# robflynnyh/long-context-asr

Measured on AMD Instinct MI355X. Metric: spectrogram-frames/sec (6L/768D, seq=16384), higher is better.
Workload: dtype bf16; 1 GPU; 6L/768D/6H SConformerXL, seq=16384, rotary theta=1.5M, fwd+CTC+bwd+clip+MADGRAD; per_gpu_batch=128, global_batch=128, seq_len=16384, parallelism=dp1

## Files before the change

long-context-asr_amd/csrc/convmod.hip:

```cpp
#include "common.h"

namespace {

constexpr int CV = 4;

struct SlabGeo {
    int cg, sl, cpb, spb;
    bool active;
    __device__ __forceinline__ SlabGeo(int CG) {
        cpb = min(64, CG); spb = 256 / cpb;
        const int cgl = threadIdx.x % cpb;
        sl = threadIdx.x / cpb;
        cg = blockIdx.y * cpb + cgl;
        active = cg < CG && sl < spb;
    }
};
template <typename AT>
__device__ __forceinline__ void slab_reduce_add(const float (&v)[CV], const SlabGeo& g, float* sh, AT* out, int d, long det_stride) {
    __syncthreads();
    if (threadIdx.x < g.cpb * g.spb) {
#pragma unroll
        for (int e = 0; e < CV; ++e) sh[g.sl * (g.cpb * CV) + (threadIdx.x % g.cpb) * CV + e] = g.active ? v[e] : 0.f;
    }
    __syncthreads();
// ... 186 lines not shown
    const long slab = (long)blockIdx.x * geo.spb + geo.sl;
    const bool live = geo.active && slab < (long)B * spb;
    const int b = live ? (int)(slab / spb) : 0, n0 = live ? (int)(slab % spb) * TN : 0;
    const int c0 = live ? geo.cg * CV : 0;
    const int L = len ? len[b] : N;
    float wk[K][CV], dhw[K][CV], aw[K][CV], gw[K][CV], gb[CV];
    float sv[CV] = {0.f, 0.f, 0.f, 0.f}, sg2[CV] = {0.f, 0.f, 0.f, 0.f};
    float mean[CV], is[CV], A[CV], Bc[CV], k0[CV], k1[CV], k2[CV];
    load4(coef + c0, mean); load4(coef + d + c0, is); load4(coef + 4 * d + c0, A); load4(coef + 5 * d + c0, Bc);
    load4(bcoef + c0, k0); load4(bcoef + d + c0, k1); load4(bcoef + 2 * d + c0, k2);
#pragma unroll
    for (int e = 0; e < CV; ++e) {
        is[e] = 1.f / is[e]; gb[e] = 0.f;
#pragma unroll
        for (int j = 0; j < K; ++j) { wk[j][e] = w[(c0 + e) * K + j]; dhw[j][e] = 0.f; aw[j][e] = 0.f; gw[j][e] = 0.f; }
    }
    const bf16* gbp = g + (long)b * N * 2 * d;
    const int nend = live ? min(N, n0 + TN) : n0 - 2 * P;
    struct Raw { bf16x4 gy, hx, va, ga, cva, cga; };
    const bf16x4 z4 = {(bf16)0.f, (bf16)0.f, (bf16)0.f, (bf16)0.f};
    auto fetch = [&](int t) {
        Raw r; r.gy = z4; r.hx = z4; r.va = z4; r.ga = z4; r.cva = z4; r.cga = z4;
        if (t >= 0 && t < N) {
            const long row = (long)b * N + t;
            r.gy = *reinterpret_cast<const bf16x4*>(dy + row * d + c0);
            r.hx = *reinterpret_cast<const bf16x4*>(h + row * d + c0);
            if (t < L) {
                r.va = *reinterpret_cast<const bf16x4*>(gbp + (long)t * 2 * d + c0);
                r.ga = *reinterpret_cast<const bf16x4*>(gbp + (long)t * 2 * d + d + c0);
            }
        }
        const int n = t - P;
        if (n >= n0 && n < nend && n < L) {
            r.cva = *reinterpret_cast<const bf16x4*>(gbp + (long)n * 2 * d + c0);
            r.cga = *reinterpret_cast<const bf16x4*>(gbp + (long)n * 2 * d + d + c0);
        }
        return r;
    };
    Raw cur = fetch(n0 - P);
    for (int t = n0 - P; t < nend + P; ++t) {
        const Raw nxt = fetch(t + 1 < nend + P ? t + 1 : -1000000);
#pragma unroll
        for (int j = 0; j < K - 1; ++j)
#pragma unroll
            for (int e = 0; e < CV; ++e) { dhw[j][e] = dhw[j + 1][e]; aw[j][e] = aw[j + 1][e]; }
        if (t >= 0 && t < N) {
#pragma unroll
            for (int e = 0; e < CV; ++e) {
                const float hx = (float)cur.hx[e];
                const float dz = (float)cur.gy[e] * dsiluf_(hx * A[e] + Bc[e]);
                dhw[K - 1][e] = k0[e] * dz - k1[e] - (hx - mean[e]) * is[e] * k2[e];
                aw[K - 1][e] = (t < L) ? (float)cur.va[e] * sigmoidf_((float)cur.ga[e]) : 0.f;
            }
        } else {
#pragma unroll
            for (int e = 0; e < CV; ++e) { dhw[K - 1][e] = 0.f; aw[K - 1][e] = 0.f; }
        }
        const int n = t - P;
        if (n >= n0 && n < nend) {
            float dv[CV], dgt[CV];
#pragma unroll
            for (int e = 0; e < CV; ++e) {
                float acc = 0.f;
                const float dhc = dhw[P][e];
#pragma unroll
                for (int j = 0; j < K; ++j) { acc += wk[j][e] * dhw[K - 1 - j][e]; gw[j][e] += dhc * aw[j][e]; }
                gb[e] += dhc;
                if (n < L) {
                    const float sg = sigmoidf_((float)cur.cga[e]);
                    dv[e] = acc * sg; dgt[e] = acc * (float)cur.cva[e] * sg * (1.f - sg);
                } else { dv[e] = 0.f; dgt[e] = 0.f; }
                sv[e] += dv[e]; sg2[e] += dgt[e];
            }
            bf16* o = dg + ((long)b * N + n) * 2 * d;
            store4(o + c0, dv); store4(o + d + c0, dgt);
        }
        cur = nxt;
    }
    slab_reduce_add<float>(gb, geo, redw, dbias, d, det_stride);
#pragma unroll
    for (int j = 0; j < K; ++j) slab_reduce_add<float>(gw[j], geo, redw, dwt + (long)j * d, d, det_stride);
    if (dgcs) { slab_reduce_add<float>(sv, geo, redw, dgcs, d, det_stride); slab_reduce_add<float>(sg2, geo, redw, dgcs + d, d, det_stride); }
}

int pick_tn(long B, long N, long CG) {
    int TN = 64;
    while (TN > 8 && B * cdiv(N, TN) * CG < 131072) TN >>= 1;
    return TN;
}

}

static dim3 glu_fwd_grid(long B, long N, long d, int& TN) {
    TN = pick_tn(B, N, d / CV);
    const int cpb = (int)std::min<long>(64, d / CV), spbk = 256 / cpb;
    return dim3(cdiv(B * cdiv(N, TN), spbk), cdiv(d / CV, cpb));
}
SCONF_API int64_t sconf_glu_dwconv_fwd_workspace(int64_t B, int64_t N, int64_t d) {
    if (B * N == 0 || d % CV != 0) return 0;
    int TN; return (int64_t)glu_fwd_grid(B, N, d, TN).x * 2 * d * 8;
}
SCONF_API int sconf_glu_dwconv_fwd(const void* g, const int32_t* lengths, const float* w, const float* bias, void* h,
                                   double* stats, void* workspace, int64_t workspace_bytes, int64_t B, int64_t N, int64_t d,
                                   int64_t ksize, hipStream_t stream) {
    SCONF_REQUIRE(d % CV == 0, "sconf_glu_dwconv_fwd: d must be a multiple of 4");
    if (B * N == 0) return 0;
    int TN;
    const dim3 grid = glu_fwd_grid(B, N, d, TN), block(256);
    SCONF_REQUIRE(ksize == 3 || ksize == 5 || ksize == 7 || ksize == 9, "sconf_glu_dwconv_fwd: unsupported kernel size %ld (3,5,7,9)", (long)ksize);
    double* sl = stats ? det_begin<double>(workspace, workspace_bytes, grid.x, 2 * d, stream) : nullptr;
    SCONF_REQUIRE(!stats || sl, "sconf_glu_dwconv_fwd: needs %ld bytes of workspace (sconf_glu_dwconv_fwd_workspace)",
                  (long)sconf_glu_dwconv_fwd_workspace(B, N, d));
#define L(KK) hipLaunchKernelGGL((glu_dwconv_fwd_kernel<KK>), grid, block, 0, stream, (const bf16*)g, lengths, w, bias, (bf16*)h, sl, (int)B, (int)N, (int)d, TN, 2 * d)
    switch (ksize) { case 3: L(3); break; case 5: L(5); break; case 7: L(7); break; default: L(9); break; }
#undef L
    if (stats) det_finish<double>(sl, grid.x, 2 * d, DetSegs<double>{{stats}, {0}, {2 * d}, 1}, stream);
    SCONF_LAUNCH_OK("sconf_glu_dwconv_fwd");
    return 0;
}

SCONF_API int sconf_brn_finalize(const double* stats, int64_t count, float* running_mean, float* running_std,
                                 int64_t* num_batches_tracked, const float* weight, const float* bias, float* coef,
                                 int64_t d, int training, float eps, float momentum, hipStream_t stream) {
    hipLaunchKernelGGL(brn_finalize_kernel, dim3(cdiv(d, 256)), dim3(256), 0, stream, stats, (double)count, running_mean,
                       running_std, (long*)num_batches_tracked, weight, bias, coef, (int)d, training, eps, momentum);
    if (training) hipLaunchKernelGGL(brn_bump_kernel, dim3(1), dim3(64), 0, stream, (long*)num_batches_tracked);
    SCONF_LAUNCH_OK("sconf_brn_finalize");
    return 0;
}

SCONF_API int sconf_affine_silu_fwd(const void* h, const float* coef, void* y, int64_t M, int64_t d, hipStream_t stream) {
    SCONF_REQUIRE(d % 8 == 0, "sconf_affine_silu_fwd: d must be a multiple of 8");
    if (M == 0) return 0;
    const int blocks = (int)std::min<long>(cdiv(M * (d / 8), 256), 8192);
    hipLaunchKernelGGL(affine_silu_fwd_kernel, dim3(blocks), dim3(256), 0, stream, (const bf16*)h, coef, (bf16*)y, (long)M, (int)d);
    SCONF_LAUNCH_OK("sconf_affine_silu_fwd");
    return 0;
}

struct ConvmodBwdGeo { int rpt, cpb, spbk, rrows, TN; dim3 grid; long gst; };
static ConvmodBwdGeo convmod_bwd_geo(long B, long N, long d, long ksize, bool colsum) {
    ConvmodBwdGeo q;
    const long M = B * N;
    const int CG = (int)(d / CV);
    q.rpt = 64;
    while (q.rpt > 8 && cdiv(M, q.rpt) * CG < 131072) q.rpt >>= 1;
    q.cpb = std::min(64, CG); q.spbk = 256 / q.cpb;
    q.rrows = cdiv(cdiv(M, q.rpt), q.spbk);
    q.TN = pick_tn(B, N, CG);
    q.grid = dim3(cdiv(B * cdiv(N, q.TN), q.spbk), cdiv(CG, q.cpb));
    q.gst = d + ksize * d + (colsum ? 2 * d : 0);
    return q;
}
SCONF_API int sconf_convmod_tile_frames(int64_t B, int64_t N, int64_t d) {
    if (B <= 0 || N <= 0 || d <= 0 || d % CV != 0) return -1;
    return pick_tn(B, N, d / CV);
}
SCONF_API int sconf_convmod_bwd_rows_per_thread(int64_t B, int64_t N, int64_t d) {
    if (B <= 0 || N <= 0 || d <= 0 || d % CV != 0) return -1;
    return convmod_bwd_geo(B, N, d, 9, false).rpt;
}
SCONF_API int64_t sconf_convmod_bwd_workspace(int64_t B, int64_t N, int64_t d, int64_t ksize, int colsum) {
    if (B * N == 0 || d % CV != 0) return 0;
    const ConvmodBwdGeo q = convmod_bwd_geo(B, N, d, ksize, colsum != 0);
    return std::max<int64_t>((int64_t)q.rrows * 2 * d * 8, (int64_t)q.grid.x * q.gst * 4);
}
SCONF_API int sconf_convmod_bwd(const void* dy, const void* h, const void* g, const int32_t* lengths, const float* w,
                                const float* brn_weight, const float* coef, double* red, float* bcoef, void* dg,
                                float* dw, float* dbias, float* dbrn_weight, float* dbrn_bias, float* dg_colsum,
                                void* workspace, int64_t workspace_bytes,
                                int64_t B, int64_t N, int64_t d, int64_t ksize, int training, float eps, hipStream_t stream) {
    SCONF_REQUIRE(d % CV == 0, "sconf_convmod_bwd: d must be a multiple of 4");
    const long M = B * N;
    if (M == 0) return 0;
    const int CG = (int)(d / CV);
    SCONF_REQUIRE(ksize == 3 || ksize == 5 || ksize == 7 || ksize == 9, "sconf_convmod_bwd: unsupported kernel size %ld (3,5,7,9)", (long)ksize);
    const ConvmodBwdGeo q = convmod_bwd_geo(B, N, d, ksize, dg_colsum != nullptr);
    const int rpt = q.rpt, cpb = q.cpb, rrows = q.rrows;
    SCONF_REQUIRE(workspace && workspace_bytes >= sconf_convmod_bwd_workspace(B, N, d, ksize, dg_colsum != nullptr),
                  "sconf_convmod_bwd: needs %ld bytes of workspace (sconf_convmod_bwd_workspace)",
                  (long)sconf_convmod_bwd_workspace(B, N, d, ksize, dg_colsum != nullptr));
    double* rsl = det_begin<double>(workspace, workspace_bytes, rrows, 2 * d, stream);
    SCONF_REQUIRE(rsl, "sconf_convmod_bwd: workspace memset failed");
    hipLaunchKernelGGL(brn_bwd_reduce_kernel, dim3(rrows, cdiv(CG, cpb)), dim3(256), 0, stream,
                       (const bf16*)dy, (const bf16*)h, coef, rsl, M, (int)d, rpt, 2 * d);
    det_finish<double>(rsl, rrows, 2 * d, DetSegs<double>{{red}, {0}, {2 * d}, 1}, stream);
    hipLaunchKernelGGL(brn_bwd_finalize_kernel, dim3(cdiv(d, 256)), dim3(256), 0, stream, red, (double)M, coef, brn_weight,
                       bcoef, dbrn_weight, dbrn_bias, (int)d, training, eps);
    const int TN = q.TN;
    const dim3 grid = q.grid, block(256);
    const long gst = q.gst;
    float* gsl = det_begin<float>(workspace, workspace_bytes, grid.x, gst, stream);
    SCONF_REQUIRE(gsl, "sconf_convmod_bwd: workspace memset failed");
#define L(KK) hipLaunchKernelGGL((dwconv_glu_bwd_kernel<KK>), grid, block, 0, stream, (const bf16*)dy, (const bf16*)h, (const bf16*)g, lengths, w, coef, bcoef, (bf16*)dg, gsl + d, gsl, dg_colsum ? gsl + d + ksize * d : nullptr, (int)B, (int)N, (int)d, TN, gst)
    switch (ksize) { case 3: L(3); break; case 5: L(5); break; case 7: L(7); break; default: L(9); break; }
#undef L
    det_finish<float>(gsl, grid.x, gst, DetSegs<float>{{dbias, dw, dg_colsum}, {0, d, d + ksize * d}, {d, ksize * d, dg_colsum ? 2 * d : 0}, dg_colsum ? 3 : 2}, stream);
    SCONF_LAUNCH_OK("sconf_convmod_bwd");
    return 0;
}
```

long-context-asr_amd/csrc/subsample.hip:

```cpp
#include "common.h"

namespace {

constexpr int CG8 = 8;


struct Geo {
    int cg, plane, c0;
    bool active;
    __device__ __forceinline__ Geo(int C, int PL) {
        const int cgs = C / CG8;
        cg = threadIdx.x % cgs; plane = threadIdx.x / cgs; c0 = cg * CG8;
        active = plane < PL;
    }
};

template <typename TX>
__global__ __launch_bounds__(256) void conv0_fwd_kernel(const TX* __restrict__ x, const float* __restrict__ w,
                                                        const float* __restrict__ bias, bf16* __restrict__ y,
                                                        int F, int T, int C, int T2, int F2, int PL, int iters) {
    const Geo g(C, PL);
    if (!g.active) return;
    const int b = blockIdx.y, npos = T2 * F2;
    float wk[9][8], bs[8];
#pragma unroll
    for (int e = 0; e < 8; ++e) { bs[e] = bias[g.c0 + e];
#pragma unroll
        for (int k = 0; k < 9; ++k) wk[k][e] = w[(g.c0 + e) * 9 + k]; }
    const TX* xb = x + (long)b * F * T;
    bf16* yb = y + (long)b * npos * C;
    for (int it = 0; it < iters; ++it) {
        const int p = (blockIdx.x * iters + it) * PL + g.plane;
        if (p >= npos) break;
        const int t2 = p / F2, f2 = p - t2 * F2;
        float in[9];
#pragma unroll
        for (int i = 0; i < 3; ++i)
#pragma unroll
            for (int j = 0; j < 3; ++j) {
                const int t = 2 * t2 + i - 1, f = 2 * f2 + j - 1;
                in[i * 3 + j] = (t >= 0 && t < T && f >= 0 && f < F) ? ld_f(xb + (long)f * T + t) : 0.f;
            }
        float o[8];
#pragma unroll
        for (int e = 0; e < 8; ++e) {
            float acc = bs[e];
#pragma unroll
            for (int k = 0; k < 9; ++k) acc += wk[k][e] * in[k];
            o[e] = acc;
        }
        store8(yb + (long)p * C + g.c0, o);
    }
}

__global__ __launch_bounds__(256) void dwconv2d_fwd_kernel(const bf16* __restrict__ x, const float* __restrict__ w,
                                                           const float* __restrict__ bias, bf16* __restrict__ y,
                                                           int Ti, int Fi, int C, int To, int Fo, int PL, int iters) {
    const Geo g(C, PL);
    if (!g.active) return;
    const int b = blockIdx.y, npos = To * Fo;
    float wk[9][8], bs[8];
#pragma unroll
    for (int e = 0; e < 8; ++e) { bs[e] = bias[g.c0 + e];
#pragma unroll
        for (int k = 0; k < 9; ++k) wk[k][e] = w[(g.c0 + e) * 9 + k]; }
    const bf16* xb = x + (long)b * Ti * Fi * C + g.c0;
    bf16* yb = y + (long)b * npos * C + g.c0;
    for (int it = 0; it < iters; ++it) {
        const int p = (blockIdx.x * iters + it) * PL + g.plane;
        if (p >= npos) break;
        const int to = p / Fo, fo = p - to * Fo;
        bf16x8 raw[9];
#pragma unroll
        for (int i = 0; i < 3; ++i)
#pragma unroll
            for (int j = 0; j < 3; ++j) {
                const int t = min(max(2 * to + i - 1, 0), Ti - 1), f = min(max(2 * fo + j - 1, 0), Fi - 1);
                raw[i * 3 + j] = *reinterpret_cast<const bf16x8*>(xb + ((long)t * Fi + f) * C);
            }
        float acc[8];
#pragma unroll
        for (int e = 0; e < 8; ++e) acc[e] = bs[e];
#pragma unroll
        for (int i = 0; i < 3; ++i)
#pragma unroll
            for (int j = 0; j < 3; ++j) {
                const int t = 2 * to + i - 1, f = 2 * fo + j - 1;
                const float in = (t >= 0 && t < Ti && f >= 0 && f < Fi) ? 1.f : 0.f;
#pragma unroll
                for (int e = 0; e < 8; ++e) acc[e] += wk[i * 3 + j][e] * (in * siluf_((float)raw[i * 3 + j][e]));
            }
        store8(yb + (long)p * C, acc);
    }
}

template <int CW>
__global__ __launch_bounds__(512) void dwconv2d_bwd_kernel(const bf16* __restrict__ dout, const float* __restrict__ w,
                                                           const bf16* __restrict__ pre_in, bf16* __restrict__ dpre_in,
                                                           float* __restrict__ dw, float* __restrict__ dbias, float* __restrict__ dcolsum,
                                                           int Ti, int Fi, int C, int To, int Fo, int PL, int iters, long det_stride) {
    __shared__ float red[512];
    {
        const long drow = ((long)blockIdx.y * gridDim.x + blockIdx.x) * det_stride;
        dw += drow; dbias += drow; if (dcolsum) dcolsum += drow;
    }
    const int cgs = C / CW;
    struct { int cg, plane, c0; bool active; } g;
    g.cg = threadIdx.x % cgs; g.plane = threadIdx.x / cgs; g.c0 = g.cg * CW; g.active = g.plane < PL;
    const int b = blockIdx.y, npos = Ti * Fi;
    float wk[9][CW], gw[9][CW], gbs[CW], gcs[CW];
#pragma unroll
    for (int e = 0; e < CW; ++e) {
        gbs[e] = 0.f; gcs[e] = 0.f;
#pragma unroll
        for (int k = 0; k < 9; ++k) { wk[k][e] = g.active ? w[(g.c0 + e) * 9 + k] : 0.f; gw[k][e] = 0.f; }
    }
    const bf16* gb = dout + (long)b * To * Fo * C + g.c0;
    const bf16* pb = pre_in + (long)b * npos * C + g.c0;
    bf16* ob = dpre_in + (long)b * npos * C + g.c0;
    if (g.active) {
        for (int it = 0; it < iters; ++it) {
            const int p = (blockIdx.x * iters + it) * PL + g.plane;
            if (p >= npos) break;
            const int ti = p / Fi, fi = p - ti * Fi;
            const int to0 = (ti + 1) >> 1, fo0 = (fi + 1) >> 1;
            float gq[2][2][CW];
#pragma unroll
            for (int a = 0; a < 2; ++a)
#pragma unroll
                for (int bb = 0; bb < 2; ++bb) {
                    const int to = min(max(to0 - a, 0), To - 1), fo = min(max(fo0 - bb, 0), Fo - 1);
                    loadv<CW>(gb + ((long)to * Fo + fo) * C, gq[a][bb]);
                }
            float pv[CW], sg[CW], sv[CW]; loadv<CW>(pb + (long)p * C, pv);
#pragma unroll
            for (int e = 0; e < CW; ++e) { sg[e] = sigmoidf_(pv[e]); sv[e] = pv[e] * sg[e]; }
            float acc[CW];
#pragma unroll
            for (int e = 0; e < CW; ++e) acc[e] = 0.f;
#pragma unroll
            for (int i = 0; i < 3; ++i) {
                const int tt = ti + 1 - i;
                if (tt < 0 || (tt & 1)) continue;
                const int to = tt >> 1;
                if (to >= To) continue;
#pragma unroll
                for (int j = 0; j < 3; ++j) {
                    const int ff = fi + 1 - j;
                    if (ff < 0 || (ff & 1)) continue;
                    const int fo = ff >> 1;
                    if (fo >= Fo) continue;
                    const float (&gv)[CW] = gq[i == 2][j == 2];
#pragma unroll
                    for (int e = 0; e < CW; ++e) {
                        acc[e] += wk[i * 3 + j][e] * gv[e];
                        gw[i * 3 + j][e] += gv[e] * sv[e];
                        if (i == 1 && j == 1) gbs[e] += gv[e];
                    }
                }
            }
#pragma unroll
            for (int e = 0; e < CW; ++e) { acc[e] *= sg[e] * (1.f + pv[e] * (1.f - sg[e])); gcs[e] += (float)(bf16)acc[e]; }
            storev<CW>(ob + (long)p * C, acc);
        }
    }
#pragma unroll
    for (int k = 0; k < 11; ++k) {
        if (k == 10 && !dcolsum) break;
#pragma unroll
        for (int e = 0; e < CW; ++e) {
            __syncthreads();
            red[threadIdx.x] = g.active ? (k < 9 ? gw[k][e] : (k == 9 ? gbs[e] : gcs[e])) : 0.f;
            __syncthreads();
            if (g.plane == 0) {
                float v = 0.f;
                for (int pl = 0; pl < PL; ++pl) v += red[pl * cgs + g.cg];
                if (k < 9) atomicAdd(dw + (g.c0 + e) * 9 + k, v); else if (k == 9) atomicAdd(dbias + g.c0 + e, v); else atomicAdd(dcolsum + g.c0 + e, v);
            }
        }
    }
}

template <bool DEPTHWISE, typename TX>
__global__ __launch_bounds__(256) void conv3x3s2_bwd_weight_kernel(const bf16* __restrict__ dout, const void* __restrict__ in_,
                                                                   float* __restrict__ dw, float* __restrict__ dbias,
                                                                   int Ti, int Fi, int C, int To, int Fo, int PL, int iters) {
    __shared__ float red[256];
    const Geo g(C, PL);
    const int cgs = C / CG8;
    const int b = blockIdx.y, npos = To * Fo;
    float gw[9][8], gbs[8];
#pragma unroll
    for (int e = 0; e < 8; ++e) { gbs[e] = 0.f;
#pragma unroll
        for (int k = 0; k < 9; ++k) gw[k][e] = 0.f; }
    const bf16* gp = dout + (long)b * npos * C + g.c0;
    if (g.active) {
        for (int it = 0; it < iters; ++it) {
            const int p = (blockIdx.x * iters + it) * PL + g.plane;
            if (p >= npos) break;
            const int to = p / Fo, fo = p - to * Fo;
            float gv[8]; load8(gp + (long)p * C, gv);
#pragma unroll
            for (int e = 0; e < 8; ++e) gbs[e] += gv[e];
#pragma unroll
            for (int i = 0; i < 3; ++i)
#pragma unroll
                for (int j = 0; j < 3; ++j) {
                    const int t = 2 * to + i - 1, f = 2 * fo + j - 1;
                    if (t < 0 || t >= Ti || f < 0 || f >= Fi) continue;
                    if (DEPTHWISE) {
                        float v[8]; load8((const bf16*)in_ + (((long)b * Ti + t) * Fi + f) * C + g.c0, v);
#pragma unroll
                        for (int e = 0; e < 8; ++e) gw[i * 3 + j][e] += gv[e] * siluf_(v[e]);
                    } else {
                        const float v = ld_f((const TX*)in_ + ((long)b * Fi + f) * Ti + t);
#pragma unroll
                        for (int e = 0; e < 8; ++e) gw[i * 3 + j][e] += gv[e] * v;
                    }
                }
        }
    }
#pragma unroll
    for (int k = 0; k < 10; ++k)
#pragma unroll
        for (int e = 0; e < 8; ++e) {
            __syncthreads();
            red[threadIdx.x] = g.active ? (k < 9 ? gw[k][e] : gbs[e]) : 0.f;
            __syncthreads();
            if (g.plane == 0) {
                float v = 0.f;
                for (int pl = 0; pl < PL; ++pl) v += red[pl * cgs + g.cg];
                if (k < 9) atomicAdd(dw + (g.c0 + e) * 9 + k, v); else atomicAdd(dbias + g.c0 + e, v);
            }
        }
}

template <bool BWD>
__global__ __launch_bounds__(256) void silu_transpose_kernel(const bf16* __restrict__ pre, const bf16* __restrict__ ds,
                                                             bf16* __restrict__ out, long rows, int F8, int C) {
    extern __shared__ __attribute__((aligned(16))) char smem_[];
    bf16* sh = reinterpret_cast<bf16*>(smem_);
    const int E = F8 * C;
    for (long row = blockIdx.x; row < rows; row += gridDim.x) {
        const bf16* pr = pre + row * E;
        if (!BWD) {
            for (int i = threadIdx.x * 8; i < E; i += 256 * 8) {
// ... 227 lines not shown
        }
    }
    fused_reduce<9>(gw0, g, C, red, dw0, 9);
    fused_reduce<1>(gb0, g, C, red, db0, 1);
    fused_reduce<9>(gwd, g, C, red, dwd, 9);
    fused_reduce<1>(gbd, g, C, red, dbd, 1);
}


struct LaunchGeo { int PL, iters, threads; dim3 grid; };
inline LaunchGeo geo_for(int64_t C, int64_t B, long npos, long target_blocks) {
    LaunchGeo g;
    const int cgs = (int)(C / 8);
    g.PL = std::max(1, 256 / cgs);
    g.threads = (cgs * g.PL + 63) / 64 * 64;
    const long per_b = std::max<long>(1, target_blocks / B);
    g.iters = (int)std::max<long>(1, cdiv(npos, (long)g.PL * per_b));
    g.grid = dim3(cdiv(npos, (long)g.PL * g.iters), (unsigned)B);
    return g;
}
#define SUB_REQ(fn) SCONF_REQUIRE(C % 8 == 0 && C / 8 <= 256, fn ": C must be a multiple of 8 and <= 2048"); \
                    SCONF_REQUIRE(B <= 65535, fn ": B must be <= 65535")

}

SCONF_API int sconf_sub_conv0_fwd(const void* x, int x_dtype, const float* w, const float* bias, void* y,
                                  int64_t B, int64_t F, int64_t T, int64_t C, hipStream_t stream) {
    SUB_REQ("sconf_sub_conv0_fwd");
    const int T2 = conv_out(T), F2 = conv_out(F);
    if (B * T2 * F2 == 0) return 0;
    const LaunchGeo g = geo_for(C, B, (long)T2 * F2, 16384);
    if (x_dtype == SCONF_F32) hipLaunchKernelGGL((conv0_fwd_kernel<float>), g.grid, dim3(g.threads), 0, stream, (const float*)x, w, bias, (bf16*)y, (int)F, (int)T, (int)C, T2, F2, g.PL, g.iters);
    else hipLaunchKernelGGL((conv0_fwd_kernel<bf16>), g.grid, dim3(g.threads), 0, stream, (const bf16*)x, w, bias, (bf16*)y, (int)F, (int)T, (int)C, T2, F2, g.PL, g.iters);
    SCONF_LAUNCH_OK("sconf_sub_conv0_fwd");
    return 0;
}

SCONF_API int sconf_sub_dwconv_fwd(const void* x, const float* w, const float* bias, void* y,
                                   int64_t B, int64_t Ti, int64_t Fi, int64_t C, hipStream_t stream) {
    SUB_REQ("sconf_sub_dwconv_fwd");
    const int To = conv_out(Ti), Fo = conv_out(Fi);
    if (B * To * Fo == 0) return 0;
    if (sconf_dwconv_window_fwd(x, w, bias, y, B, Ti, Fi, C, stream)) { SCONF_LAUNCH_OK("sconf_sub_dwconv_fwd"); return 0; }
    const LaunchGeo g = geo_for(C, B, (long)To * Fo, 16384);
    hipLaunchKernelGGL(dwconv2d_fwd_kernel, g.grid, dim3(g.threads), 0, stream, (const bf16*)x, w, bias, (bf16*)y, (int)Ti, (int)Fi, (int)C, To, Fo, g.PL, g.iters);
    SCONF_LAUNCH_OK("sconf_sub_dwconv_fwd");
    return 0;
}

struct DwBwdGeo { int cw, PL, threads, iters; dim3 grid; };
static DwBwdGeo dwconv_bwd_geo(long B, long Ti, long Fi, long C) {
    DwBwdGeo q;
    long target = 512; int cw = 8;
    if (const char* e = getenv("SCONF_SUB_DWBWD_CFG")) { int a = 0; long t = 0; if (sscanf(e, "%d,%ld", &a, &t) == 2) { cw = a; target = t; } }
    const int cgs = (int)(C / cw);
    int nthr = 256;
    if (const char* e = getenv("SCONF_SUB_DWBWD_THREADS")) { const int v = atoi(e); if (v == 256 || v == 512) nthr = v; }
    q.cw = cw;
    q.PL = std::max(1, nthr / cgs); q.threads = (cgs * q.PL + 63) / 64 * 64;
    const long npos = (long)Ti * Fi, per_b = std::max<long>(1, target / B);
    q.iters = (int)std::max<long>(1, cdiv(npos, (long)q.PL * per_b));
    q.grid = dim3(cdiv(npos, (long)q.PL * q.iters), (unsigned)B);
    return q;
}
SCONF_API int64_t sconf_sub_dwconv_bwd_workspace(int64_t B, int64_t Ti, int64_t Fi, int64_t C, int colsum) {
    if (B * Ti * Fi == 0 || C <= 0) return 0;
    const DwBwdGeo q = dwconv_bwd_geo(B, Ti, Fi, C);
    return (int64_t)q.grid.x * q.grid.y * (10 * C + (colsum ? C : 0)) * 4;
}
SCONF_API int sconf_sub_dwconv_bwd(const void* dout, const float* w, const void* pre_in, void* dpre_in, float* dw, float* dbias,
                                   float* dpre_colsum, void* workspace, int64_t workspace_bytes, int64_t B, int64_t Ti, int64_t Fi,
                                   int64_t C, hipStream_t stream) {
    SUB_REQ("sconf_sub_dwconv_bwd");
    const int To = conv_out(Ti), Fo = conv_out(Fi);
    if (B * Ti * Fi == 0) return 0;
    const DwBwdGeo q = dwconv_bwd_geo(B, Ti, Fi, C);
    SCONF_REQUIRE(C / q.cw <= 256, "sconf_sub_dwconv_bwd: C too large");
    const int cw = q.cw, PL = q.PL, threads = q.threads, iters = q.iters;
    const dim3 grid = q.grid;
    const long rows = (long)grid.x * grid.y, dst = 10 * C + (dpre_colsum ? C : 0);
    float* sl = det_begin<float>(workspace, workspace_bytes, rows, dst, stream);
    SCONF_REQUIRE(sl, "sconf_sub_dwconv_bwd: needs %ld bytes of workspace (sconf_sub_dwconv_bwd_workspace)", rows * dst * 4);
    float* scs = dpre_colsum ? sl + 10 * C : nullptr;
    if (cw == 8) hipLaunchKernelGGL((dwconv2d_bwd_kernel<8>), grid, dim3(threads), 0, stream, (const bf16*)dout, w, (const bf16*)pre_in, (bf16*)dpre_in, sl, sl + 9 * C, scs, (int)Ti, (int)Fi, (int)C, To, Fo, PL, iters, dst);
    else         hipLaunchKernelGGL((dwconv2d_bwd_kernel<4>), grid, dim3(threads), 0, stream, (const bf16*)dout, w, (const bf16*)pre_in, (bf16*)dpre_in, sl, sl + 9 * C, scs, (int)Ti, (int)Fi, (int)C, To, Fo, PL, iters, dst);
    det_finish<float>(sl, rows, dst, DetSegs<float>{{dw, dbias, dpre_colsum}, {0, 9 * C, 10 * C}, {9 * C, C, dpre_colsum ? C : 0}, dpre_colsum ? 3 : 2}, stream);
    SCONF_LAUNCH_OK("sconf_sub_dwconv_bwd");
    return 0;
}

SCONF_API int sconf_sub_conv0_bwd(const void* dpre0, const void* x, int x_dtype, float* dw, float* dbias,
                                  int64_t B, int64_t F, int64_t T, int64_t C, hipStream_t stream) {
    SUB_REQ("sconf_sub_conv0_bwd");
    const int T2 = conv_out(T), F2 = conv_out(F);
    if (B * T2 * F2 == 0) return 0;
    const LaunchGeo g = geo_for(C, B, (long)T2 * F2, 1024);
    if (x_dtype == SCONF_F32) hipLaunchKernelGGL((conv3x3s2_bwd_weight_kernel<false, float>), g.grid, dim3(g.threads), 0, stream, (const bf16*)dpre0, x, dw, dbias, (int)T, (int)F, (int)C, T2, F2, g.PL, g.iters);
    else hipLaunchKernelGGL((conv3x3s2_bwd_weight_kernel<false, bf16>), g.grid, dim3(g.threads), 0, stream, (const bf16*)dpre0, x, dw, dbias, (int)T, (int)F, (int)C, T2, F2, g.PL, g.iters);
    SCONF_LAUNCH_OK("sconf_sub_conv0_bwd");
    return 0;
}

SCONF_API int sconf_sub_silu_transpose(int bwd, const void* pre, const void* ds, void* out, int64_t rows, int64_t F8, int64_t C,
                                       hipStream_t stream) {
    SCONF_REQUIRE(C % 8 == 0, "sconf_sub_silu_transpose: C must be a multiple of 8");
    SCONF_REQUIRE(F8 * C * 2 <= 64 * 1024, "sconf_sub_silu_transpose: row of %ld elements does not fit LDS", (long)(F8 * C));
    if (rows == 0) return 0;
    const int blocks = (int)std::min<long>(rows, 8192);
    const size_t sh = (size_t)F8 * C * 2;
    if (!bwd) hipLaunchKernelGGL((silu_transpose_kernel<false>), dim3(blocks), dim3(256), sh, stream, (const bf16*)pre, (const bf16*)ds, (bf16*)out, (long)rows, (int)F8, (int)C);
    else      hipLaunchKernelGGL((silu_transpose_kernel<true>), dim3(blocks), dim3(256), sh, stream, (const bf16*)pre, (const bf16*)ds, (bf16*)out, (long)rows, (int)F8, (int)C);
    SCONF_LAUNCH_OK("sconf_sub_silu_transpose");
    return 0;
}

SCONF_API int sconf_sub_stage01_fwd(const void* x, int x_dtype, const float* w0, const float* b0, const float* wd, const float* bd,
                                    void* d1, int64_t B, int64_t F, int64_t T, int64_t C, hipStream_t stream) {
    SCONF_REQUIRE(C % 4 == 0 && C / 4 <= 256, "sconf_sub_stage01_fwd: C must be a multiple of 4 and <= 1024");
    SCONF_REQUIRE(B <= 65535 && F <= 1024, "sconf_sub_stage01_fwd: B <= 65535 and F <= 1024");
    const int T2 = conv_out(T), F2 = conv_out(F), T4 = conv_out(T2), F4 = conv_out(F2);
    if (B * T4 * F4 == 0) return 0;
    if (sconf_stage01_fwd_mfma(x, x_dtype, w0, b0, wd, bd, d1, B, F, T, C, stream)) { SCONF_LAUNCH_OK("sconf_sub_stage01_fwd"); return 0; }
    const long target = env_long("SCONF_SUB_FWD_BLOCKS", 4096);
    const int rpb = std::max(1, (int)cdiv((long)T4 * B, target));
    dim3 grid(cdiv(T4, rpb), (unsigned)B), block(512);
    const size_t sh = (size_t)7 * F * 4 + (size_t)3 * F2 * C * 2;
    SCONF_REQUIRE(sh <= 150 * 1024, "sconf_sub_stage01_fwd: the 3-row activation window (%ld B) does not fit LDS", (long)sh);
    static bool attr_set = false;
    lds_limit_once(attr_set, {(const void*)stage01_fwd_kernel<float>, (const void*)stage01_fwd_kernel<bf16>}, 150 * 1024);
    if (x_dtype == SCONF_F32) hipLaunchKernelGGL((stage01_fwd_kernel<float>), grid, block, sh, stream, (const float*)x, w0, b0, wd, bd, (bf16*)d1, (int)F, (int)T, (int)C, T2, F2, T4, F4, rpb);
    else hipLaunchKernelGGL((stage01_fwd_kernel<bf16>), grid, block, sh, stream, (const bf16*)x, w0, b0, wd, bd, (bf16*)d1, (int)F, (int)T, (int)C, T2, F2, T4, F4, rpb);
    SCONF_LAUNCH_OK("sconf_sub_stage01_fwd");
    return 0;
}

SCONF_API int sconf_sub_stage01_slabs(int64_t F, int64_t C, int bwd) { return stage01_mfma_slabs(F, C, bwd); }

SCONF_API int64_t sconf_sub_stage01_bwd_workspace(int64_t B, int64_t F, int64_t T, int64_t C) { return stage01_bwd_mfma_workspace(B, F, T, C); }
SCONF_API int sconf_sub_stage01_bwd(const void* dd1, const void* x, int x_dtype, const float* w0, const float* b0, const float* wd,
                                    float* dw0, float* db0, float* dwd, float* dbd, void* workspace, int64_t workspace_bytes,
                                    int64_t B, int64_t F, int64_t T, int64_t C, hipStream_t stream) {
    SCONF_REQUIRE(C % 4 == 0 && C / 4 <= 256, "sconf_sub_stage01_bwd: C must be a multiple of 4 and <= 1024");
    SCONF_REQUIRE(B <= 65535 && F <= 1024, "sconf_sub_stage01_bwd: B <= 65535 and F <= 1024");
    const int T2 = conv_out(T), F2 = conv_out(F), T4 = conv_out(T2), F4 = conv_out(F2);
    if (B * T4 * F4 == 0) return 0;
    const int mf = sconf_stage01_bwd_mfma(dd1, x, x_dtype, w0, b0, wd, dw0, db0, dwd, dbd, workspace, workspace_bytes, B, F, T, C, stream);
    if (mf < 0) return 1;
    if (mf) { SCONF_LAUNCH_OK("sconf_sub_stage01_bwd"); return 0; }
    int rw = 4; long target = 512;
    if (const char* e = getenv("SCONF_SUB_BWD_CFG")) { int a = 0; long t = 0; if (sscanf(e, "%d,%ld", &a, &t) == 2) { rw = a; target = t; } }
    auto lds_bytes = [&](int r) { return (size_t)((2 * r + 1) * F + 256) * 4 + (size_t)(r / 2 + 2) * F4 * C * 2; };
    while (rw > 1 && lds_bytes(rw) > 64 * 1024) rw /= 2;
    int rpb2 = std::max(1, (int)cdiv((long)T2 * B, target));
    rpb2 = (rpb2 + rw - 1) / rw * rw;
    dim3 g2(cdiv(T2, rpb2), (unsigned)B), block(256);
    const size_t sh = lds_bytes(rw);
    SCONF_REQUIRE(sh <= 64 * 1024 && (F4 * C) % 8 == 0, "sconf_sub_stage01_bwd: dd1 rows do not fit LDS");
#define LB(TX, RW_) hipLaunchKernelGGL((stage01_bwd_kernel<TX, RW_>), g2, block, sh, stream, (const TX*)x, w0, b0, wd, (const bf16*)dd1, dw0, db0, dwd, dbd, (int)F, (int)T, (int)C, T2, F2, T4, F4, rpb2)
    if (x_dtype == SCONF_F32) { if (rw == 1) LB(float, 1); else if (rw == 4) LB(float, 4); else LB(float, 2); }
    else                      { if (rw == 1) LB(bf16, 1); else if (rw == 4) LB(bf16, 4); else LB(bf16, 2); }
#undef LB
    SCONF_LAUNCH_OK("sconf_sub_stage01_bwd");
    return 0;
}
```

Measured before the change: 7.164 million spectrogram-frames/sec.

## Stream conv backward inputs through LDS rings via async buffer loads

Adds ring-buffered variants of the depthwise-conv GLU backward kernel (K=9) and the subsampling 2D depthwise-conv backward kernel. Each wave issues direct buffer-to-LDS loads several steps ahead and reads operands from shared memory, so global loads overlap with compute instead of stalling on per-iteration loads. The new paths need extra dynamic LDS per block, which can lower occupancy, and they rely on 32-bit buffer offsets, so they are guarded by size checks.

```diff
diff --git a/long-context-asr_amd/csrc/convmod.hip b/long-context-asr_amd/csrc/convmod.hip
--- a/long-context-asr_amd/csrc/convmod.hip
+++ b/long-context-asr_amd/csrc/convmod.hip
@@ -292,6 +292,146 @@
     for (int j = 0; j < K; ++j) slab_reduce_add<float>(gw[j], geo, redw, dwt + (long)j * d, d, det_stride);
     if (dgcs) { slab_reduce_add<float>(sv, geo, redw, dgcs, d, det_stride); slab_reduce_add<float>(sg2, geo, redw, dgcs + d, d, det_stride); }
 }
+
+constexpr int GL_AHEAD = 3;
+template <int K> constexpr int gl_gslots() { return GL_AHEAD + ((K - 1) / 2 + 1) / 2; }
+template <int K> constexpr int gl_wave_bytes() { return (GL_AHEAD + gl_gslots<K>()) * 2048; }
+template <int K>
+__global__ __launch_bounds__(256) void dwconv_glu_bwd_ring_kernel(const bf16* __restrict__ dy, const bf16* __restrict__ h,
+                                                                  const bf16* __restrict__ g, const int* __restrict__ len,
+                                                                  const float* __restrict__ w, const float* __restrict__ coef,
+                                                                  const float* __restrict__ bcoef, bf16* __restrict__ dg,
+                                                                  float* __restrict__ dwt, float* __restrict__ dbias,
+                                                                  float* __restrict__ dgcs, int B, int N, int d, int TN, long det_stride) {
+    extern __shared__ __attribute__((aligned(16))) unsigned char ring[];
+    constexpr int P = (K - 1) / 2;
+    __shared__ float redw[1024];
+    const int CG = d / CV, spb = (N + TN - 1) / TN;
+    const SlabGeo geo(CG);
+    const long slab = (long)blockIdx.x * geo.spb + geo.sl;
+    const bool live = geo.active && slab < (long)B * spb;
+    const int b = live ? (int)(slab / spb) : 0, n0 = live ? (int)(slab % spb) * TN : 0;
+    const int c0 = live ? geo.cg * CV : 0;
+    const int L = len ? len[b] : N;
+    float wk[K][CV], dhw[K][CV], aw[K][CV], gw[K][CV], gb[CV];
+    float sv[CV] = {0.f, 0.f, 0.f, 0.f}, sg2[CV] = {0.f, 0.f, 0.f, 0.f};
+    float mean[CV], is[CV], A[CV], Bc[CV], k0[CV], k1[CV], k2[CV];
+    load4(coef + c0, mean); load4(coef + d + c0, is); load4(coef + 4 * d + c0, A); load4(coef + 5 * d + c0, Bc);
+    load4(bcoef + c0, k0); load4(bcoef + d + c0, k1); load4(bcoef + 2 * d + c0, k2);
+#pragma unroll
+    for (int e = 0; e < CV; ++e) {
+        is[e] = 1.f / is[e]; gb[e] = 0.f;
+#pragma unroll
+        for (int j = 0; j < K; ++j) { wk[j][e] = w[(c0 + e) * K + j]; dhw[j][e] = 0.f; aw[j][e] = 0.f; gw[j][e] = 0.f; }
+    }
+    const int nend = live ? min(N, n0 + TN) : n0 - 2 * P;
+    struct Raw { bf16x4 gy, hx, va, ga, cva, cga; };
+    constexpr int NG = gl_gslots<K>();
+    const int wave = __builtin_amdgcn_readfirstlane((int)(threadIdx.x >> 6)), lane = threadIdx.x & 63;
+    const int bu = __builtin_amdgcn_readfirstlane(b), t0 = __builtin_amdgcn_readfirstlane(n0 - P);
+    const int tend = __builtin_amdgcn_readfirstlane(nend + P);
+    const unsigned char* mx = ring + wave * gl_wave_bytes<K>() + lane * 8;
+    const unsigned char* mg = mx + GL_AHEAD * 2048;
+    const unsigned rx = lds_addr(ring) + wave * gl_wave_bytes<K>(), rg = rx + GL_AHEAD * 2048;
+    const srd_t sy = make_srd(dy + (long)bu * N * d, (long)N * d * 2), sh = make_srd(h + (long)bu * N * d, (long)N * d * 2);
+    const srd_t sgl = make_srd(g + (long)bu * N * 2 * d, (long)N * d * 4);
+    const unsigned inrow = blockIdx.y * (64 * CV * 2) + (lane & 31) * 16;
+    const unsigned vx = (lane >> 5) * (unsigned)d * 2 + inrow, vg = (lane >> 5) * (unsigned)d * 4 + inrow;
+    auto issue = [&](int q, unsigned xs_, unsigned gs_) {
+        const unsigned ox = (unsigned)((t0 + 2 * q) * d * 2);
+        dma_piece(sy, vx + ox, 0u, rx + xs_);
+        dma_piece(sh, vx + ox, 0u, rx + xs_ + 1024);
+        dma_piece(sgl, vg + 2 * ox, 0u, rg + gs_);
+        dma_piece(sgl, vg + 2 * ox + (unsigned)d * 2, 0u, rg + gs_ + 1024);
+    };
+#pragma unroll
+    for (int e = 0; e < CV; ++e) {
+        tie(mean[e]); tie(is[e]); tie(A[e]); tie(Bc[e]); tie(k0[e]); tie(k1[e]); tie(k2[e]);
+#pragma unroll
+        for (int j = 0; j < K; ++j) tie(wk[j][e]);
+    }
+    if (t0 < tend) {
+#pragma unroll
+        for (int q = 0; q < GL_AHEAD; ++q) issue(q, q * 2048, q * 2048);
+    }
+    int r = 0;
+    unsigned xs = 0, gs = 0, gi = GL_AHEAD * 2048, cs = 0;
+    bool full = false;
+    auto fetch = [&]() {
+        const int f = r & 1, fc = (r - P) & 1;
+        if (!f) wait_vm<4 * (GL_AHEAD - 1)>();
+        Raw v;
+        v.gy = *reinterpret_cast<const bf16x4*>(mx + xs + f * 512);
+        v.hx = *reinterpret_cast<const bf16x4*>(mx + xs + 1024 + f * 512);
+        v.va = *reinterpret_cast<const bf16x4*>(mg + gs + f * 512);
+        v.ga = *reinterpret_cast<const bf16x4*>(mg + gs + 1024 + f * 512);
+        v.cva = *reinterpret_cast<const bf16x4*>(mg + cs + fc * 512);
+        v.cga = *reinterpret_cast<const bf16x4*>(mg + cs + 1024 + fc * 512);
+        if (r >= P && fc) cs = cs + 2048 == NG * 2048 ? 0 : cs + 2048;
+        full = f;
+        ++r;
+        return v;
+    };
+    auto recycle = [&]() {
+        if (full) {
+            wait_lgkm0();
+            issue((r >> 1) - 1 + GL_AHEAD, xs, gi);
+            xs = xs + 2048 == GL_AHEAD * 2048 ? 0 : xs + 2048;
+            gs = gs + 2048 == NG * 2048 ? 0 : gs + 2048;
+            gi = gi + 2048 == NG * 2048 ? 0 : gi + 2048;
+        }
+    };
+    Raw cur = fetch();
+#pragma unroll 1
+    for (int t = t0; t < tend; ++t) {
+        const Raw nxt = fetch();
+#pragma unroll
+        for (int j = 0; j < K - 1; ++j)
+#pragma unroll
+            for (int e = 0; e < CV; ++e) { dhw[j][e] = dhw[j + 1][e]; aw[j][e] = aw[j + 1][e]; }
+        if (t >= 0 && t < N) {
+#pragma unroll
+            for (int e = 0; e < CV; ++e) {
+                const float hx = (float)cur.hx[e];
+                const float dz = (float)cur.gy[e] * dsiluf_(hx * A[e] + Bc[e]);
+                dhw[K - 1][e] = k0[e] * dz - k1[e] - (hx - mean[e]) * is[e] * k2[e];
+                aw[K - 1][e] = (t < L) ? (float)cur.va[e] * sigmoidf_((float)cur.ga[e]) : 0.f;
+            }
+        } else {
+#pragma unroll
+            for (int e = 0; e < CV; ++e) { dhw[K - 1][e] = 0.f; aw[K - 1][e] = 0.f; }
+        }
+        const int n = t - P;
+        if (n >= n0 && n < nend) {
+            float dv[CV], dgt[CV];
+#pragma unroll
+            for (int e = 0; e < CV; ++e) {
+                float acc = 0.f;
+                const float dhc = dhw[P][e];
+#pragma unroll
+                for (int j = 0; j < K; ++j) { acc += wk[j][e] * dhw[K - 1 - j][e]; gw[j][e] += dhc * aw[j][e]; }
+                gb[e] += dhc;
+                if (n < L) {
+                    const float sg = sigmoidf_((float)cur.cga[e]);
+                    dv[e] = acc * sg; dgt[e] = acc * (float)cur.cva[e] * sg * (1.f - sg);
+                } else { dv[e] = 0.f; dgt[e] = 0.f; }
+                sv[e] += dv[e]; sg2[e] += dgt[e];
+            }
+            if (live) {
+                bf16* o = dg + ((long)b * N + n) * 2 * d;
+                store4(o + c0, dv); store4(o + d + c0, dgt);
+            }
+        }
+        recycle();
+        cur = nxt;
+    }
+    wait_vm<0>();
+    slab_reduce_add<float>(gb, geo, redw, dbias, d, det_stride);
+#pragma unroll
+    for (int j = 0; j < K; ++j) slab_reduce_add<float>(gw[j], geo, redw, dwt + (long)j * d, d, det_stride);
+    if (dgcs) { slab_reduce_add<float>(sv, geo, redw, dgcs, d, det_stride); slab_reduce_add<float>(sg2, geo, redw, dgcs + d, d, det_stride); }
+}
+
 
 int pick_tn(long B, long N, long CG) {
     int TN = 64;
@@ -402,9 +542,15 @@
     const long gst = q.gst;
     float* gsl = det_begin<float>(workspace, workspace_bytes, grid.x, gst, stream);
     SCONF_REQUIRE(gsl, "sconf_convmod_bwd: workspace memset failed");
+    if (ksize == 9 && cpb == 64 && N * d * 4 < (1L << 30)) {
+        const size_t rsh = (size_t)4 * gl_wave_bytes<9>();
+        static bool attr = false; lds_limit_once(attr, {(const void*)dwconv_glu_bwd_ring_kernel<9>}, rsh);
+        hipLaunchKernelGGL((dwconv_glu_bwd_ring_kernel<9>), grid, block, rsh, stream, (const bf16*)dy, (const bf16*)h, (const bf16*)g, lengths, w, coef, bcoef, (bf16*)dg, gsl + d, gsl, dg_colsum ? gsl + d + ksize * d : nullptr, (int)B, (int)N, (int)d, TN, gst);
+    } else {
 #define L(KK) hipLaunchKernelGGL((dwconv_glu_bwd_kernel<KK>), grid, block, 0, stream, (const bf16*)dy, (const bf16*)h, (const bf16*)g, lengths, w, coef, bcoef, (bf16*)dg, gsl + d, gsl, dg_colsum ? gsl + d + ksize * d : nullptr, (int)B, (int)N, (int)d, TN, gst)
-    switch (ksize) { case 3: L(3); break; case 5: L(5); break; case 7: L(7); break; default: L(9); break; }
+        switch (ksize) { case 3: L(3); break; case 5: L(5); break; case 7: L(7); break; default: L(9); break; }
 #undef L
+    }
     det_finish<float>(gsl, grid.x, gst, DetSegs<float>{{dbias, dw, dg_colsum}, {0, d, d + ksize * d}, {d, ksize * d, dg_colsum ? 2 * d : 0}, dg_colsum ? 3 : 2}, stream);
     SCONF_LAUNCH_OK("sconf_convmod_bwd");
     return 0;
diff --git a/long-context-asr_amd/csrc/subsample.hip b/long-context-asr_amd/csrc/subsample.hip
--- a/long-context-asr_amd/csrc/subsample.hip
+++ b/long-context-asr_amd/csrc/subsample.hip
@@ -94,12 +94,16 @@
     }
 }
 
-template <int CW>
+constexpr int DW_RING = 3;
+constexpr int DW_SLOT = 5 * 1024;
+template <int CW, bool RING>
 __global__ __launch_bounds__(512) void dwconv2d_bwd_kernel(const bf16* __restrict__ dout, const float* __restrict__ w,
                                                            const bf16* __restrict__ pre_in, bf16* __restrict__ dpre_in,
                                                            float* __restrict__ dw, float* __restrict__ dbias, float* __restrict__ dcolsum,
                                                            int Ti, int Fi, int C, int To, int Fo, int PL, int iters, long det_stride) {
+    static_assert(!RING || CW == 8, "the ring moves 16-byte pieces");
     __shared__ float red[512];
+    extern __shared__ __attribute__((aligned(16))) unsigned char ring[];
     {
         const long drow = ((long)blockIdx.y * gridDim.x + blockIdx.x) * det_stride;
         dw += drow; dbias += drow; if (dcolsum) dcolsum += drow;
@@ -118,51 +122,110 @@
     const bf16* gb = dout + (long)b * To * Fo * C + g.c0;
     const bf16* pb = pre_in + (long)b * npos * C + g.c0;
     bf16* ob = dpre_in + (long)b * npos * C + g.c0;
-    if (g.active) {
-        for (int it = 0; it < iters; ++it) {
+    auto position = [&](int p, int ti, int fi, const float (&gq)[2][2][CW], const float (&pv)[CW]) {
+        float sg[CW], sv[CW];
+#pragma unroll
+        for (int e = 0; e < CW; ++e) { sg[e] = sigmoidf_(pv[e]); sv[e] = pv[e] * sg[e]; }
+        float acc[CW];
+#pragma unroll
+        for (int e = 0; e < CW; ++e) acc[e] = 0.f;
+#pragma unroll
+        for (int i = 0; i < 3; ++i) {
+            const int tt = ti + 1 - i;
+            if (tt < 0 || (tt & 1)) continue;
+            const int to = tt >> 1;
+            if (to >= To) continue;
+#pragma unroll
+            for (int j = 0; j < 3; ++j) {
+                const int ff = fi + 1 - j;
+                if (ff < 0 || (ff & 1)) continue;
+                const int fo = ff >> 1;
+                if (fo >= Fo) continue;
+                const float (&gv)[CW] = gq[i == 2][j == 2];
+#pragma unroll
+                for (int e = 0; e < CW; ++e) {
+                    acc[e] += wk[i * 3 + j][e] * gv[e];
+                    gw[i * 3 + j][e] += gv[e] * sv[e];
+                    if (i == 1 && j == 1) gbs[e] += gv[e];
+                }
+            }
+        }
+#pragma unroll
+        for (int e = 0; e < CW; ++e) {
+            if constexpr (RING) {
+#pragma clang fp reassociate(off)
+                acc[e] = (acc[e] * sg[e]) * (1.f + pv[e] * (1.f - sg[e]));
+            } else acc[e] *= sg[e] * (1.f + pv[e] * (1.f - sg[e]));
+            gcs[e] += (float)(bf16)acc[e];
+        }
+        storev<CW>(ob + (long)p * C, acc);
+    };
+    if constexpr (!RING) {
+        if (g.active) {
+            for (int it = 0; it < iters; ++it) {
+                const int p = (blockIdx.x * iters + it) * PL + g.plane;
+                if (p >= npos) break;
+                const int ti = p / Fi, fi = p - ti * Fi;
+                const int to0 = (ti + 1) >> 1, fo0 = (fi + 1) >> 1;
+                float gq[2][2][CW];
+#pragma unroll
+                for (int a = 0; a < 2; ++a)
+#pragma unroll
+                    for (int bb = 0; bb < 2; ++bb) {
+                        const int to = min(max(to0 - a, 0), To - 1), fo = min(max(fo0 - bb, 0), Fo - 1);
+                        loadv<CW>(gb + ((long)to * Fo + fo) * C, gq[a][bb]);
+                    }
+                float pv[CW]; loadv<CW>(pb + (long)p * C, pv);
+                position(p, ti, fi, gq, pv);
+            }
+        }
+    } else {
+        const int wave = __builtin_amdgcn_readfirstlane((int)(threadIdx.x >> 6));
+        const unsigned char* mine = ring + wave * (DW_RING * DW_SLOT) + (threadIdx.x & 63) * 16;
+        const unsigned ring0 = lds_addr(ring) + wave * (DW_RING * DW_SLOT);
+        const srd_t sp = make_srd(pre_in + (long)b * npos * C, (long)npos * C * 2);
+        const srd_t sd = make_srd(dout + (long)b * To * Fo * C, (long)To * Fo * C * 2);
+        const unsigned step = (unsigned)PL * C * 2;
+        const unsigned vp = (unsigned)blockIdx.x * iters * step + threadIdx.x * 16;
+        auto issue = [&](int it, unsigned slot) {
             const int p = (blockIdx.x * iters + it) * PL + g.plane;
-            if (p >= npos) break;
             const int ti = p / Fi, fi = p - ti * Fi;
             const int to0 = (ti + 1) >> 1, fo0 = (fi + 1) >> 1;
-            float gq[2][2][CW];
+            dma_piece(sp, vp + (unsigned)it * step, 0u, ring0 + slot);
 #pragma unroll
             for (int a = 0; a < 2; ++a)
 #pragma unroll
                 for (int bb = 0; bb < 2; ++bb) {
                     const int to = min(max(to0 - a, 0), To - 1), fo = min(max(fo0 - bb, 0), Fo - 1);
-                    loadv<CW>(gb + ((long)to * Fo + fo) * C, gq[a][bb]);
+                    dma_piece(sd, (unsigned)(((to * Fo + fo) * C + g.c0) * 2), 0u, ring0 + slot + (1 + a * 2 + bb) * 1024);
                 }
-            float pv[CW], sg[CW], sv[CW]; loadv<CW>(pb + (long)p * C, pv);
-#pragma unroll
-            for (int e = 0; e < CW; ++e) { sg[e] = sigmoidf_(pv[e]); sv[e] = pv[e] * sg[e]; }
-            float acc[CW];
-#pragma unroll
-            for (int e = 0; e < CW; ++e) acc[e] = 0.f;
-#pragma unroll
-            for (int i = 0; i < 3; ++i) {
-                const int tt = ti + 1 - i;
-                if (tt < 0 || (tt & 1)) continue;
-                const int to = tt >> 1;
-                if (to >= To) continue;
-#pragma unroll
-                for (int j = 0; j < 3; ++j) {
-                    const int ff = fi + 1 - j;
-                    if (ff < 0 || (ff & 1)) continue;
-                    const int fo = ff >> 1;
-                    if (fo >= Fo) continue;
-                    const float (&gv)[CW] = gq[i == 2][j == 2];
-#pragma unroll
-                    for (int e = 0; e < CW; ++e) {
-                        acc[e] += wk[i * 3 + j][e] * gv[e];
-                        gw[i * 3 + j][e] += gv[e] * sv[e];
-                        if (i == 1 && j == 1) gbs[e] += gv[e];
-                    }
-                }
-            }
-#pragma unroll
-            for (int e = 0; e < CW; ++e) { acc[e] *= sg[e] * (1.f + pv[e] * (1.f - sg[e])); gcs[e] += (float)(bf16)acc[e]; }
-            storev<CW>(ob + (long)p * C, acc);
-        }
+        };
+#pragma unroll
+        for (int e = 0; e < CW; ++e)
+#pragma unroll
+            for (int k = 0; k < 9; ++k) tie(wk[k][e]);
+#pragma unroll
+        for (int k = 0; k < DW_RING; ++k) issue(k, k * DW_SLOT);
+        unsigned slot = 0;
+        for (int it = 0; it < iters; ++it) {
+            if ((blockIdx.x * iters + it) * PL + (wave * 64) / cgs >= npos) break;
+            wait_vm<5 * (DW_RING - 1)>();
+            const int p = (blockIdx.x * iters + it) * PL + g.plane;
+            if (g.active && p < npos) {
+                const int ti = p / Fi, fi = p - ti * Fi;
+                float gq[2][2][CW];
+#pragma unroll
+                for (int a = 0; a < 2; ++a)
+#pragma unroll
+                    for (int bb = 0; bb < 2; ++bb) load8(reinterpret_cast<const bf16*>(mine + slot + (1 + a * 2 + bb) * 1024), gq[a][bb]);
+                float pv[CW]; load8(reinterpret_cast<const bf16*>(mine + slot), pv);
+                position(p, ti, fi, gq, pv);
+            }
+            wait_lgkm0();
+            issue(it + DW_RING, slot);
+            slot = slot + DW_SLOT == DW_RING * DW_SLOT ? 0 : slot + DW_SLOT;
+        }
+        wait_vm<0>();
     }
 #pragma unroll
     for (int k = 0; k < 11; ++k) {
@@ -556,8 +619,14 @@
     float* sl = det_begin<float>(workspace, workspace_bytes, rows, dst, stream);
     SCONF_REQUIRE(sl, "sconf_sub_dwconv_bwd: needs %ld bytes of workspace (sconf_sub_dwconv_bwd_workspace)", rows * dst * 4);
     float* scs = dpre_colsum ? sl + 10 * C : nullptr;
-    if (cw == 8) hipLaunchKernelGGL((dwconv2d_bwd_kernel<8>), grid, dim3(threads), 0, stream, (const bf16*)dout, w, (const bf16*)pre_in, (bf16*)dpre_in, sl, sl + 9 * C, scs, (int)Ti, (int)Fi, (int)C, To, Fo, PL, iters, dst);
-    else         hipLaunchKernelGGL((dwconv2d_bwd_kernel<4>), grid, dim3(threads), 0, stream, (const bf16*)dout, w, (const bf16*)pre_in, (bf16*)dpre_in, sl, sl + 9 * C, scs, (int)Ti, (int)Fi, (int)C, To, Fo, PL, iters, dst);
+#define LD(CW_, RING_, SH_) hipLaunchKernelGGL((dwconv2d_bwd_kernel<CW_, RING_>), grid, dim3(threads), SH_, stream, (const bf16*)dout, w, (const bf16*)pre_in, (bf16*)dpre_in, sl, sl + 9 * C, scs, (int)Ti, (int)Fi, (int)C, To, Fo, PL, iters, dst)
+    if (cw == 8 && Ti * Fi * C * 2 < (1L << 30)) {
+        const size_t sh = (size_t)(threads / 64) * DW_RING * DW_SLOT;
+        if (sh > 48 * 1024) { static bool attr = false; lds_limit_once(attr, {(const void*)dwconv2d_bwd_kernel<8, true>}, (size_t)8 * DW_RING * DW_SLOT); }
+        LD(8, true, sh);
+    } else if (cw == 8) LD(8, false, 0);
+    else LD(4, false, 0);
+#undef LD
     det_finish<float>(sl, rows, dst, DetSegs<float>{{dw, dbias, dpre_colsum}, {0, 9 * C, 10 * C}, {9 * C, C, dpre_colsum ? C : 0}, dpre_colsum ? 3 : 2}, stream);
     SCONF_LAUNCH_OK("sconf_sub_dwconv_bwd");
     return 0;
```

Measured after the change: 7.188 million spectrogram-frames/sec (median of 6 runs). About the same (+0.3%).
